# NUS-HPC-AI-Lab/VideoSys

Hardware: AMD Instinct MI355X
Metric: videos/min (Open-Sora 512x512x64f, 30 denoise steps, DiT denoising only) + sec/denoise-step (higher is better)
Workload: dtype bf16

## Files before the change

### videosys_amd/csrc/gemm2_bf16.hip

```cpp
#include "common.h"
#include "vsys_internal.h"

namespace vsys {
namespace {

constexpr int BM = 256, BK = 32;
constexpr int A_SLOT = BM * BK * 2;
constexpr int W_BASE = 3 * A_SLOT;
constexpr int OUT_ROW_BYTES = 96 * 2 + 16;
constexpr int OUT_WAVE_BYTES = 64 * OUT_ROW_BYTES;

template <int NWN>
struct G2 {
  static constexpr int NW = 2 * NWN;
  static constexpr int NT = 64 * NW;
  static constexpr int BN = 96 * NWN;
  static constexpr int NA = 16 / NW;
  static constexpr int W_SLOT = BN * BK * 2;
  static constexpr int WLEAD = NWN == 4 ? 2 : 1;
  static constexpr int NWSLOT = WLEAD + 1;
  static constexpr int STAGING = W_BASE + NWSLOT * W_SLOT;
  static constexpr int LDS_BYTES = STAGING > NW * OUT_WAVE_BYTES ? STAGING : NW * OUT_WAVE_BYTES;
  static constexpr int LN_BYTES = (BM + BN) * 8;
};

template <int EPI, int NWN, int STAMP = 0, int MF = 0>
__global__ __launch_bounds__(G2<NWN>::NT, 2) void gemm2_kernel(GemmParams p) {
  using G = G2<NWN>;
  constexpr int BN = G::BN, NA = G::NA, W_SLOT = G::W_SLOT, WLEAD = G::WLEAD;
#if __HIP_DEVICE_COMPILE__
  extern __shared__ __attribute__((aligned(16))) char smem[];
  const int tid = threadIdx.x, lane = tid & 63, wave = tid >> 6;
  const int wm = wave / NWN, wn = wave % NWN;
  const int l31 = lane & 31, hi = lane >> 5;
  const int l15 = lane & 15, lq = lane >> 4;
  static_assert(!MF || (EPI != EPI_F32_SLICES && !STAMP), "the 16x16x32 form covers the token-row epilogues only");
  const int wave_u = __builtin_amdgcn_readfirstlane(wave);
  const int nbn = p.N / BN;
  int tile = xcd_remap(blockIdx.x, gridDim.x);
  int kslice = 0;
  if constexpr (EPI == EPI_F32_SLICES) {
    const int ntile = ((p.M + BM - 1) / BM) * nbn;
    kslice = tile / ntile;
    tile -= kslice * ntile;
  }
  int bm, bn;
  gemm_raster(tile, (p.M + BM - 1) / BM, nbn, p.raster_gw, p.raster_ph, bm, bn);
  const int row0 = bm * BM, col0 = bn * BN;

  const int dchunk = ((lane & 3) ^ (MF ? ((0x78 >> (2 * ((lane >> 4) & 3))) & 3) : ((lane >> 4) & 3))) * 16;
  int a_off[NA], b_off[3];
#pragma unroll
  for (int i = 0; i < NA; ++i) {
    const int r = wave_u * (16 * NA) + i * 16 + (lane >> 2);
    const int rl = row0 + r < p.M ? r : p.M - 1 - row0;
    a_off[i] = rl * (int)p.lda * 2 + dchunk;
  }
#pragma unroll
  for (int i = 0; i < 3; ++i) b_off[i] = (wave_u * 48 + i * 16 + (lane >> 2)) * (int)p.ldw * 2 + dchunk;
  const int64_t a_bytes = ((int64_t)(p.M - 1 - row0) * p.lda + p.K) * 2, b_bytes = ((int64_t)(p.N - 1 - col0) * p.ldw + p.K) * 2;
  const auto rsrc_a = __builtin_amdgcn_make_buffer_rsrc((void*)(p.A + (int64_t)row0 * p.lda), 0,
                                                        (int)(a_bytes < 0x7fffffff ? a_bytes : 0x7fffffff), 0x00020000);
  const auto rsrc_b = __builtin_amdgcn_make_buffer_rsrc((void*)(p.W + (int64_t)col0 * p.ldw), 0,
                                                        (int)(b_bytes < 0x7fffffff ? b_bytes : 0x7fffffff), 0x00020000);
  typedef __attribute__((address_space(3))) void* lds_ptr_t;
  const int kbase2 = EPI == EPI_F32_SLICES ? kslice * p.ks * 2 : 0;
  auto dma_a = [&](int i, int t, int slot) {
    __builtin_amdgcn_raw_ptr_buffer_load_lds(rsrc_a, (lds_ptr_t)(smem + slot * A_SLOT + (wave_u * (16 * NA) + i * 16) * 64), 16, a_off[i],
                                             kbase2 + t * (BK * 2), 0, 0);
  };
  auto dma_w = [&](int i, int t, int slot) {
    __builtin_amdgcn_raw_ptr_buffer_load_lds(rsrc_b, (lds_ptr_t)(smem + W_BASE + slot * W_SLOT + (wave_u * 48 + i * 16) * 64), 16,
                                             b_off[i], kbase2 + t * (BK * 2), 0, 0);
  };

  const int fsw = MF ? ((lq ^ ((0x78 >> (2 * ((l15 >> 2) & 3))) & 3)) << 4) : ((hi ^ ((l31 >> 2) & 3)) << 4);
  const int frow = MF ? l15 : l31;
  const int xo = (wm * 128 + frow) * 64 + fsw;
  const int wo = W_BASE + (wn * 96 + frow) * 64 + fsw;

  f32x16 acc[MF ? 1 : 4][MF ? 1 : 3];
  f32x4 acc16[MF ? 8 : 1][MF ? 6 : 1];
#pragma unroll
  for (int i = 0; i < (MF ? 1 : 4); ++i)
#pragma unroll
    for (int j = 0; j < (MF ? 1 : 3); ++j)
#pragma unroll
      for (int r = 0; r < 16; ++r) acc[i][j][r] = 0.f;
#pragma unroll
  for (int i = 0; i < (MF ? 8 : 1); ++i)
#pragma unroll
    for (int j = 0; j < (MF ? 6 : 1); ++j)
#pragma unroll
      for (int r = 0; r < 4; ++r) acc16[i][j][r] = 0.f;

  constexpr bool LN = EPI == EPI_LN_BIAS || EPI == EPI_LN_GELU;
  float2* ln_lds = reinterpret_cast<float2*>(smem + G::LDS_BYTES);
  const int nt = (EPI == EPI_F32_SLICES ? (p.ks < p.K - kslice * p.ks ? p.ks : p.K - kslice * p.ks) : p.K) / BK;
#pragma unroll
  for (int i = 0; i < NA; ++i) dma_a(i, 0, 0);
#pragma unroll
  for (int i = 0; i < 3; ++i) dma_w(i, 0, 0);
  if (nt > 1) {
#pragma unroll
    for (int i = 0; i < NA; ++i) dma_a(i, 1, 1);
    if constexpr (WLEAD == 2) {
#pragma unroll
      for (int i = 0; i < 3; ++i) dma_w(i, 1, 1);
    }
  }
  if constexpr (LN) {
    __builtin_amdgcn_sched_barrier(0);
    ln_stage_tile(ln_lds, p.ln_stats, p.ln_ld, p.ln_nb, p.ln_eps, p.M, row0, BM, p.cs, p.cv, col0, BN, tid, G::NT);
    __builtin_amdgcn_sched_barrier(0);
  }
  if (nt > 1) {
    if constexpr (WLEAD == 2) {
      asm volatile("s_waitcnt vmcnt(5)" ::: "memory");
    } else if constexpr (NA == 4) {
      asm volatile("s_waitcnt vmcnt(4)" ::: "memory");
    } else {
      asm volatile("s_waitcnt vmcnt(2)" ::: "memory");
    }
  } else {
    asm volatile("s_waitcnt vmcnt(0)" ::: "memory");
  }
  if constexpr (LN) asm volatile("s_waitcnt lgkmcnt(0)" ::: "memory");
  __builtin_amdgcn_sched_barrier(0);
  __builtin_amdgcn_s_barrier();
  __builtin_amdgcn_sched_barrier(0);

  int sa = 0, sw = 0;
  uint64_t st_read = 0, st_mfma = 0, st_wait = 0, st_bar = 0, st_t0 = 0, st_begin = 0;
  if constexpr (STAMP) { st_begin = __builtin_amdgcn_s_memtime(); st_t0 = st_begin; }
  for (int t = 0; t < nt; ++t) {
    const int sa1 = sa == 2 ? 0 : sa + 1, sa2 = sa1 == 2 ? 0 : sa1 + 1;
    const int sw1 = WLEAD == 2 ? sa1 : (sw ^ 1);
    const int swn = WLEAD == 2 ? sa2 : sw1;
    const int tw = t + WLEAD;
    const bool n2 = t + 2 < nt;
    const bool n1 = WLEAD == 2 ? n2 : (t + 1 < nt);
    const char* ab = smem + sa * A_SLOT;
    const char* wb = smem + sw * W_SLOT;
    bf16x8 x0, x1, x2, x3, w0, w1, w2, v0, v1, v2;
    if constexpr (MF) {
      x0 = *reinterpret_cast<const bf16x8*>(ab + xo);
      w0 = *reinterpret_cast<const bf16x8*>(wb + wo);
      w1 = *reinterpret_cast<const bf16x8*>(wb + wo + 1024);
      w2 = *reinterpret_cast<const bf16x8*>(wb + wo + 2048);
      v0 = *reinterpret_cast<const bf16x8*>(wb + wo + 3072);
      v1 = *reinterpret_cast<const bf16x8*>(wb + wo + 4096);
      v2 = *reinterpret_cast<const bf16x8*>(wb + wo + 5120);
      x1 = *reinterpret_cast<const bf16x8*>(ab + xo + 1024);
      x2 = *reinterpret_cast<const bf16x8*>(ab + xo + 2048);
      x3 = *reinterpret_cast<const bf16x8*>(ab + xo + 3072);
      __builtin_amdgcn_sched_barrier(0);
#define G16_ROW(i_, X_)                                                                                \
  acc16[i_][0] = __builtin_amdgcn_mfma_f32_16x16x32_bf16(w0, X_, acc16[i_][0], 0, 0, 0);               \
  acc16[i_][1] = __builtin_amdgcn_mfma_f32_16x16x32_bf16(w1, X_, acc16[i_][1], 0, 0, 0);               \
  acc16[i_][2] = __builtin_amdgcn_mfma_f32_16x16x32_bf16(w2, X_, acc16[i_][2], 0, 0, 0);               \
  acc16[i_][3] = __builtin_amdgcn_mfma_f32_16x16x32_bf16(v0, X_, acc16[i_][3], 0, 0, 0);               \
  acc16[i_][4] = __builtin_amdgcn_mfma_f32_16x16x32_bf16(v1, X_, acc16[i_][4], 0, 0, 0);               \
  acc16[i_][5] = __builtin_amdgcn_mfma_f32_16x16x32_bf16(v2, X_, acc16[i_][5], 0, 0, 0)
      G16_ROW(0, x0);
      __builtin_amdgcn_sched_barrier(0);
      x0 = *reinterpret_cast<const bf16x8*>(ab + xo + 4096);
      if (n1) { dma_w(0, tw, swn); dma_w(1, tw, swn); }
      __builtin_amdgcn_sched_barrier(0);
      G16_ROW(1, x1);
      __builtin_amdgcn_sched_barrier(0);
      x1 = *reinterpret_cast<const bf16x8*>(ab + xo + 5120);
      if (n1) dma_w(2, tw, swn);
      if (n2) dma_a(0, t + 2, sa2);
      __builtin_amdgcn_sched_barrier(0);
      G16_ROW(2, x2);
      __builtin_amdgcn_sched_barrier(0);
      x2 = *reinterpret_cast<const bf16x8*>(ab + xo + 6144);
      if (n2) {
        dma_a(1, t + 2, sa2);
        if constexpr (NA > 2) dma_a(2 < NA ? 2 : 0, t + 2, sa2);
      }
      __builtin_amdgcn_sched_barrier(0);
      G16_ROW(3, x3);
      __builtin_amdgcn_sched_barrier(0);
      x3 = *reinterpret_cast<const bf16x8*>(ab + xo + 7168);
      if constexpr (NA > 3) {
        if (n2) dma_a(3 < NA ? 3 : 0, t + 2, sa2);
      }
      __builtin_amdgcn_sched_barrier(0);
      G16_ROW(4, x0);
      G16_ROW(5, x1);
      G16_ROW(6, x2);
      G16_ROW(7, x3);
#undef G16_ROW
    } else {
    x0 = *reinterpret_cast<const bf16x8*>(ab + xo);
    w0 = *reinterpret_cast<const bf16x8*>(wb + wo);
    w1 = *reinterpret_cast<const bf16x8*>(wb + wo + 2048);
    w2 = *reinterpret_cast<const bf16x8*>(wb + wo + 4096);
    x1 = *reinterpret_cast<const bf16x8*>(ab + xo + 2048);
    x2 = *reinterpret_cast<const bf16x8*>(ab + xo + 4096);
    x3 = *reinterpret_cast<const bf16x8*>(ab + xo + 6144);
    v0 = *reinterpret_cast<const bf16x8*>(wb + (wo ^ 32));
    v1 = *reinterpret_cast<const bf16x8*>(wb + (wo ^ 32) + 2048);
    v2 = *reinterpret_cast<const bf16x8*>(wb + (wo ^ 32) + 4096);
    __builtin_amdgcn_sched_barrier(0);
    if constexpr (STAMP) {
      asm volatile("s_waitcnt lgkmcnt(0)" ::: "memory");
      const uint64_t now = __builtin_amdgcn_s_memtime();
      st_read += now - st_t0; st_t0 = now;
      __builtin_amdgcn_sched_barrier(0);
    }
#define G2_ROW(i_, X_, W0_, W1_, W2_)                                                                  \
  acc[i_][0] = __builtin_amdgcn_mfma_f32_32x32x16_bf16(W0_, X_, acc[i_][0], 0, 0, 0);                  \
  acc[i_][1] = __builtin_amdgcn_mfma_f32_32x32x16_bf16(W1_, X_, acc[i_][1], 0, 0, 0);                  \
  acc[i_][2] = __builtin_amdgcn_mfma_f32_32x32x16_bf16(W2_, X_, acc[i_][2], 0, 0, 0)
    G2_ROW(0, x0, w0, w1, w2);
    __builtin_amdgcn_sched_barrier(0);
    x0 = *reinterpret_cast<const bf16x8*>(ab + (xo ^ 32));
    if (n1) { dma_w(0, tw, swn); dma_w(1, tw, swn); }
    __builtin_amdgcn_sched_barrier(0);
    G2_ROW(1, x1, w0, w1, w2);
    __builtin_amdgcn_sched_barrier(0);
    x1 = *reinterpret_cast<const bf16x8*>(ab + (xo ^ 32) + 2048);
    if (n1) dma_w(2, tw, swn);
    if (n2) dma_a(0, t + 2, sa2);
    __builtin_amdgcn_sched_barrier(0);
    G2_ROW(2, x2, w0, w1, w2);
    __builtin_amdgcn_sched_barrier(0);
    x2 = *reinterpret_cast<const bf16x8*>(ab + (xo ^ 32) + 4096);
    if (n2) {
      dma_a(1, t + 2, sa2);
      if constexpr (NA > 2) dma_a(2 < NA ? 2 : 0, t + 2, sa2);
    }
    __builtin_amdgcn_sched_barrier(0);
    G2_ROW(3, x3, w0, w1, w2);
    __builtin_amdgcn_sched_barrier(0);
    x3 = *reinterpret_cast<const bf16x8*>(ab + (xo ^ 32) + 6144);
    if constexpr (NA > 3) {
      if (n2) dma_a(3 < NA ? 3 : 0, t + 2, sa2);
    }
    __builtin_amdgcn_sched_barrier(0);
    G2_ROW(0, x0, v0, v1, v2);
    G2_ROW(1, x1, v0, v1, v2);
    G2_ROW(2, x2, v0, v1, v2);
    G2_ROW(3, x3, v0, v1, v2);
#undef G2_ROW
    }
    __builtin_amdgcn_sched_barrier(0);
    if constexpr (STAMP) {
      const uint64_t now = __builtin_amdgcn_s_memtime();
      st_mfma += now - st_t0; st_t0 = now;
      __builtin_amdgcn_sched_barrier(0);
    }
    if (n2) {
      if constexpr (WLEAD == 2) asm volatile("s_waitcnt vmcnt(5) lgkmcnt(0)" ::: "memory");
      else if constexpr (NA == 4) asm volatile("s_waitcnt vmcnt(4) lgkmcnt(0)" ::: "memory");
      else asm volatile("s_waitcnt vmcnt(2) lgkmcnt(0)" ::: "memory");
    } else {
      asm volatile("s_waitcnt vmcnt(0) lgkmcnt(0)" ::: "memory");
    }
    __builtin_amdgcn_sched_barrier(0);
    if constexpr (STAMP) {
      const uint64_t now = __builtin_amdgcn_s_memtime();
      st_wait += now - st_t0; st_t0 = now;
      __builtin_amdgcn_sched_barrier(0);
    }
    __builtin_amdgcn_s_barrier();
    __builtin_amdgcn_sched_barrier(0);
    if constexpr (STAMP) {
      const uint64_t now = __builtin_amdgcn_s_memtime();
      st_bar += now - st_t0; st_t0 = now;
      __builtin_amdgcn_sched_barrier(0);
    }
    sa = sa1;
    sw = sw1;
  }

  if constexpr (EPI == EPI_F32_SLICES) {
    float* o32 = p.out32 + (int64_t)kslice * p.slab;
    const int ncol0 = col0 + wn * 96;
#pragma unroll
    for (int i = 0; i < 4; ++i) {
      const int n = row0 + wm * 128 + i * 32 + l31;
      if (n < p.M) {
#pragma unroll
        for (int j = 0; j < 3; ++j)
#pragma unroll
          for (int g = 0; g < 4; ++g)
#pragma unroll
            for (int r = 0; r < 4; ++r) {
              const int m = ncol0 + j * 32 + 8 * g + 4 * hi + r;
              if (m < p.rows_per_sample) o32[(int64_t)m * p.ldo32 + n] = acc[i][j][4 * g + r];
            }
      }
    }
    return;
  }
  char* st = smem + wave * OUT_WAVE_BYTES;
  const int ncol0 = col0 + wn * 96;
  uint2 bb[3][4];
#pragma unroll
  for (int j = 0; j < 3; ++j)
#pragma unroll
    for (int g = 0; g < 4; ++g) bb[j][g] = make_uint2(0, 0);
  if (p.bias != nullptr && EPI != EPI_LN_BIAS && EPI != EPI_LN_GELU && !MF) {
#pragma unroll
    for (int j = 0; j < 3; ++j)
#pragma unroll
      for (int g = 0; g < 4; ++g) bb[j][g] = *reinterpret_cast<const uint2*>(p.bias + ncol0 + j * 32 + 8 * g + 4 * hi);
  }
  uint2 bb16[6];
#pragma unroll
  for (int j = 0; j < 6; ++j) bb16[j] = make_uint2(0, 0);
  if (MF && p.bias != nullptr && EPI != EPI_LN_BIAS && EPI != EPI_LN_GELU) {
#pragma unroll
    for (int j = 0; j < 6; ++j) bb16[j] = *reinterpret_cast<const uint2*>(p.bias + ncol0 + j * 16 + 4 * lq);
  }
  const bool full = row0 + BM <= p.M;
#pragma unroll
  for (int ih = 0; ih < 2; ++ih) {
    const int wrow0 = row0 + wm * 128 + ih * 64;
    if constexpr (MF) {
      if constexpr (LN) {
        float mu[4], rs[4];
#pragma unroll
        for (int i2 = 0; i2 < 4; ++i2) {
          const float2 ms = ln_lds[wm * 128 + ih * 64 + i2 * 16 + l15];
          mu[i2] = ms.x;
          rs[i2] = ms.y;
        }
#pragma unroll
        for (int j = 0; j < 6; ++j) {
          const float4* cp = reinterpret_cast<const float4*>(ln_lds + BM + wn * 96 + j * 16 + 4 * lq);
          const float4 a = cp[0], b = cp[1];
          const float c_s[4] = {a.x, a.z, b.x, b.z}, c_v[4] = {a.y, a.w, b.y, b.w};
#pragma unroll
          for (int i2 = 0; i2 < 4; ++i2) {
            const int i = ih * 4 + i2;
            const float nmu = -mu[i2], r_ = rs[i2];
            float v[4];
#pragma unroll
            for (int r = 0; r < 4; ++r) v[r] = fmaf(r_, fmaf(nmu, c_s[r], acc16[i][j][r]), c_v[r]);
            if (EPI == EPI_LN_GELU) {
#pragma unroll
              for (int r = 0; r < 4; ++r) v[r] = gelu_tanh(v[r]);
            }
            uint2 o;
            o.x = pack2bf(v[0], v[1]);
            o.y = pack2bf(v[2], v[3]);
            *reinterpret_cast<uint2*>(st + (i2 * 16 + l15) * OUT_ROW_BYTES + (j * 16 + 4 * lq) * 2) = o;
          }
        }
      } else {
        constexpr bool GATED16 = EPI == EPI_GATE_RES || EPI == EPI_GATE_RES_STATS;
        if (GATED16 && p.res != nullptr) {
#pragma unroll
          for (int half = 0; half < 2; ++half) {
            uint4 r6[6];
#pragma unroll
            for (int k = 0; k < 6; ++k) {
              const int q = lane + 64 * (6 * half + k);
              const int m_local = q / 12, c = q - m_local * 12;
              int grow = wrow0 + m_local;
              grow = grow < p.M ? grow : p.M - 1;
              r6[k] = *reinterpret_cast<const uint4*>(p.res + (int64_t)grow * p.ldr + ncol0 + c * 8);
            }
#pragma unroll
            for (int k = 0; k < 6; ++k) {
              const int q = lane + 64 * (6 * half + k);
              const int m_local = q / 12, c = q - m_local * 12;
              *reinterpret_cast<uint4*>(st + m_local * OUT_ROW_BYTES + c * 16) = r6[k];
            }
          }
          asm volatile("s_waitcnt lgkmcnt(0)" ::: "memory");
          __builtin_amdgcn_wave_barrier();
        }
#pragma unroll
        for (int i2 = 0; i2 < 4; ++i2) {
          const int i = ih * 4 + i2;
          const int m_local = i2 * 16 + l15;
          const bf16_t* gate_row = nullptr;
          if (GATED16 && p.gate != nullptr) {
            int grow = wrow0 + m_local;
            grow = grow < p.M ? grow : p.M - 1;
            const int sample = grow / p.rows_per_sample;
            gate_row = p.gate + (int64_t)sample * p.gate_stride + ncol0 + 4 * lq;
            if (p.seg_split > 0 && grow - sample * p.rows_per_sample < p.seg_split) gate_row += p.gate_alt;
          }
#pragma unroll
          for (int j = 0; j < 6; ++j) {
            uint2 gg = make_uint2(0x3f803f80u, 0x3f803f80u);
            if (GATED16 && gate_row != nullptr) gg = *reinterpret_cast<const uint2*>(gate_row + j * 16);
            float v[4];
#pragma unroll
            for (int r = 0; r < 4; ++r) v[r] = acc16[i][j][r];
            v[0] += bflo(bb16[j].x); v[1] += bfhi(bb16[j].x); v[2] += bflo(bb16[j].y); v[3] += bfhi(bb16[j].y);
            if (EPI == EPI_BIAS_GELU) {
#pragma unroll
              for (int r = 0; r < 4; ++r) v[r] = gelu_tanh(v[r]);
            }
            if (GATED16) {
              v[0] *= bflo(gg.x); v[1] *= bfhi(gg.x); v[2] *= bflo(gg.y); v[3] *= bfhi(gg.y);
            }
            uint2 o;
            o.x = pack2bf(v[0], v[1]);
            o.y = pack2bf(v[2], v[3]);
            if (GATED16 && p.res != nullptr) {
              const uint2 rr = *reinterpret_cast<const uint2*>(st + m_local * OUT_ROW_BYTES + (j * 16 + 4 * lq) * 2);
              o.x = pack2bf(bflo(o.x) + bflo(rr.x), bfhi(o.x) + bfhi(rr.x));
              o.y = pack2bf(bflo(o.y) + bflo(rr.y), bfhi(o.y) + bfhi(rr.y));
            }
            *reinterpret_cast<uint2*>(st + m_local * OUT_ROW_BYTES + (j * 16 + 4 * lq) * 2) = o;
          }
        }
        if constexpr (EPI == EPI_GATE_RES_STATS) {
          asm volatile("s_waitcnt lgkmcnt(0)" ::: "memory");
          __builtin_amdgcn_wave_barrier();
#pragma unroll
          for (int i2 = 0; i2 < 2; ++i2) {
            const int m_local = i2 * 32 + l31;
            LnAcc lacc;
#pragma unroll
            for (int j = 0; j < 3; ++j)
#pragma unroll
              for (int g = 0; g < 4; ++g) {
                const uint2 o = *reinterpret_cast<const uint2*>(st + m_local * OUT_ROW_BYTES + (j * 32 + 8 * g + 4 * hi) * 2);
                if (j == 0 && g == 0) lacc.init(bflo(o.x));
                lacc.add(bflo(o.x)); lacc.add(bfhi(o.x)); lacc.add(bflo(o.y)); lacc.add(bfhi(o.y));
              }
            const float2 mine = lacc.finish(48.f);
            const float2 other = make_float2(__shfl_xor(mine.x, 32, 64), __shfl_xor(mine.y, 32, 64));
            const float2 blk = ln_merge_equal(mine, other, 48.f);
            const int grow = wrow0 + m_local;
            if (hi == 0 && grow < p.M) p.stats_out[(int64_t)(ncol0 / LN_BLOCK) * p.stats_ld + grow] = blk;
          }
        }
      }
    } else {
    if constexpr (LN) {
      float mu[2], rs[2];
#pragma unroll
      for (int i2 = 0; i2 < 2; ++i2) {
        const float2 ms = ln_lds[wm * 128 + ih * 64 + i2 * 32 + l31];
        mu[i2] = ms.x;
        rs[i2] = ms.y;
      }
#pragma unroll
      for (int j = 0; j < 3; ++j) {
        float4 c_s[4], c_v[4];
#pragma unroll
        for (int g = 0; g < 4; ++g) {
          const float4* cp = reinterpret_cast<const float4*>(ln_lds + BM + wn * 96 + j * 32 + 8 * g + 4 * hi);
          const float4 a = cp[0], b = cp[1];
          c_s[g] = make_float4(a.x, a.z, b.x, b.z);
          c_v[g] = make_float4(a.y, a.w, b.y, b.w);
        }
#pragma unroll
        for (int i2 = 0; i2 < 2; ++i2) {
          const int i = ih * 2 + i2;
          const int m_local = i2 * 32 + l31;
          const float nmu = -mu[i2], r_ = rs[i2];
#pragma unroll
          for (int g = 0; g < 4; ++g) {
            const int n_local = j * 32 + 8 * g + 4 * hi;
            float v[4];
            v[0] = fmaf(r_, fmaf(nmu, c_s[g].x, acc[i][j][4 * g + 0]), c_v[g].x);
            v[1] = fmaf(r_, fmaf(nmu, c_s[g].y, acc[i][j][4 * g + 1]), c_v[g].y);
            v[2] = fmaf(r_, fmaf(nmu, c_s[g].z, acc[i][j][4 * g + 2]), c_v[g].z);
            v[3] = fmaf(r_, fmaf(nmu, c_s[g].w, acc[i][j][4 * g + 3]), c_v[g].w);
            if (EPI == EPI_LN_GELU) {
#pragma unroll
              for (int r = 0; r < 4; ++r) v[r] = gelu_tanh(v[r]);
            }
            uint2 o;
            o.x = pack2bf(v[0], v[1]);
            o.y = pack2bf(v[2], v[3]);
            *reinterpret_cast<uint2*>(st + m_local * OUT_ROW_BYTES + n_local * 2) = o;
          }
        }
      }
    }
#pragma unroll
    for (int i2 = 0; i2 < (LN ? 0 : 2); ++i2) {
      const int i = ih * 2 + i2;
      const int m_local = i2 * 32 + l31;
      const bf16_t* gate_row = nullptr;
      if (EPI == EPI_GATE_RES && p.gate != nullptr) {
        int grow = wrow0 + m_local;
        grow = grow < p.M ? grow : p.M - 1;
        const int sample = grow / p.rows_per_sample;
        gate_row = p.gate + (int64_t)sample * p.gate_stride + ncol0 + 4 * hi;
        if (p.seg_split > 0 && grow - sample * p.rows_per_sample < p.seg_split) gate_row += p.gate_alt;
      }
#pragma unroll
      for (int j = 0; j < 3; ++j) {
        uint2 gg[4];
        if (EPI == EPI_GATE_RES) {
#pragma unroll
          for (int g = 0; g < 4; ++g) gg[g] = make_uint2(0x3f803f80u, 0x3f803f80u);
          if (gate_row != nullptr) {
#pragma unroll
            for (int g = 0; g < 4; ++g) gg[g] = *reinterpret_cast<const uint2*>(gate_row + j * 32 + 8 * g);
          }
        }
#pragma unroll
        for (int g = 0; g < 4; ++g) {
          const int n_local = j * 32 + 8 * g + 4 * hi;
          float v[4];
#pragma unroll
          for (int r = 0; r < 4; ++r) v[r] = acc[i][j][4 * g + r];
          v[0] += bflo(bb[j][g].x); v[1] += bfhi(bb[j][g].x); v[2] += bflo(bb[j][g].y); v[3] += bfhi(bb[j][g].y);
          if (EPI == EPI_BIAS_GELU) {
#pragma unroll
            for (int r = 0; r < 4; ++r) v[r] = gelu_tanh(v[r]);
          }
          if (EPI == EPI_GATE_RES) {
            v[0] *= bflo(gg[g].x); v[1] *= bfhi(gg[g].x); v[2] *= bflo(gg[g].y); v[3] *= bfhi(gg[g].y);
          }
          uint2 o;
          o.x = pack2bf(v[0], v[1]);
          o.y = pack2bf(v[2], v[3]);
          *reinterpret_cast<uint2*>(st + m_local * OUT_ROW_BYTES + n_local * 2) = o;
        }
      }
    }
    }
    uint4 rres[12];
    if (EPI == EPI_GATE_RES && !MF) {
#pragma unroll
      for (int it = 0; it < 12; ++it) rres[it] = make_uint4(0, 0, 0, 0);
      if (p.res != nullptr) {
#pragma unroll
        for (int it = 0; it < 12; ++it) {
          const int q = lane + 64 * it;
          const int m_local = q / 12, c = q - m_local * 12;
          int grow = wrow0 + m_local;
          grow = grow < p.M ? grow : p.M - 1;
          rres[it] = *reinterpret_cast<const uint4*>(p.res + (int64_t)grow * p.ldr + ncol0 + c * 8);
        }
      }
    }
    asm volatile("s_waitcnt lgkmcnt(0)" ::: "memory");
    __builtin_amdgcn_wave_barrier();
    uint4 val[12];
#pragma unroll
    for (int it = 0; it < 12; ++it) {
      const int q = lane + 64 * it;
      const int m_local = q / 12, c = q - m_local * 12;
      val[it] = *reinterpret_cast<const uint4*>(st + m_local * OUT_ROW_BYTES + c * 16);
    }
#pragma unroll
    for (int it = 0; it < 12; ++it) {
      const int q = lane + 64 * it;
      const int m_local = q / 12, c = q - m_local * 12;
      const int64_t grow = wrow0 + m_local;
      const int gcol = ncol0 + c * 8;
      const bool ok = full || grow < p.M;
      uint4 v = val[it];
      if (EPI == EPI_GATE_RES && !MF) {
        if (p.aux != nullptr && ok) *reinterpret_cast<uint4*>(p.aux + grow * p.ldaux + gcol) = v;
        if (p.res != nullptr) {
          float a[8], b[8];
          unpack8(v, a);
          unpack8(rres[it], b);
#pragma unroll
          for (int e = 0; e < 8; ++e) a[e] += b[e];
          v = pack8(a);
        }
      }
      if (ok) *reinterpret_cast<uint4*>(p.out + grow * p.ldo + gcol) = v;
    }
    asm volatile("s_waitcnt lgkmcnt(0)" ::: "memory");
    __builtin_amdgcn_wave_barrier();
  }
  if constexpr (STAMP) {
    if (lane == 0 && p.aux != nullptr) {
      int64_t* d = reinterpret_cast<int64_t*>(p.aux) + ((int64_t)blockIdx.x * G::NW + wave) * 8;
      const uint64_t end = __builtin_amdgcn_s_memtime();
      d[0] = (int64_t)st_read; d[1] = (int64_t)st_mfma; d[2] = (int64_t)st_wait; d[3] = (int64_t)st_bar;
      d[4] = (int64_t)(st_t0 - st_begin); d[5] = (int64_t)(end - st_t0); d[6] = (int64_t)st_begin; d[7] = nt;
    }
  }
#endif
}

}

template <int NWN, int MF = 0>
static int launch_gemm2_t(const GemmParams& p, int epi, hipStream_t stream) {
  using G = G2<NWN>;
  if (p.N % G::BN != 0) return VSYS_ERR_SHAPE;
  const int nbm = (p.M + BM - 1) / BM, nbn = p.N / G::BN;
  const int grid = nbm * nbn;
  static std::atomic<unsigned long long> attr_seen{0};
  for (DeviceOnce once(attr_seen); once.todo(); once.done()) {
    (void)hipFuncSetAttribute((const void*)gemm2_kernel<EPI_BIAS, NWN, 0, MF>, hipFuncAttributeMaxDynamicSharedMemorySize, G::LDS_BYTES);
    (void)hipFuncSetAttribute((const void*)gemm2_kernel<EPI_BIAS_GELU, NWN, 0, MF>, hipFuncAttributeMaxDynamicSharedMemorySize, G::LDS_BYTES);
    (void)hipFuncSetAttribute((const void*)gemm2_kernel<EPI_GATE_RES, NWN, 0, MF>, hipFuncAttributeMaxDynamicSharedMemorySize, G::LDS_BYTES);
    (void)hipFuncSetAttribute((const void*)gemm2_kernel<EPI_LN_BIAS, NWN, 0, MF>, hipFuncAttributeMaxDynamicSharedMemorySize, G::LDS_BYTES + G::LN_BYTES);
    (void)hipFuncSetAttribute((const void*)gemm2_kernel<EPI_LN_GELU, NWN, 0, MF>, hipFuncAttributeMaxDynamicSharedMemorySize, G::LDS_BYTES + G::LN_BYTES);
    if constexpr (MF)
      (void)hipFuncSetAttribute((const void*)gemm2_kernel<EPI_GATE_RES_STATS, NWN, 0, MF>, hipFuncAttributeMaxDynamicSharedMemorySize, G::LDS_BYTES);
  }
  switch (epi) {
    case EPI_LN_BIAS: hipLaunchKernelGGL((gemm2_kernel<EPI_LN_BIAS, NWN, 0, MF>), dim3(grid), dim3(G::NT), G::LDS_BYTES + G::LN_BYTES, stream, p); break;
    case EPI_LN_GELU: hipLaunchKernelGGL((gemm2_kernel<EPI_LN_GELU, NWN, 0, MF>), dim3(grid), dim3(G::NT), G::LDS_BYTES + G::LN_BYTES, stream, p); break;
    case EPI_BIAS: hipLaunchKernelGGL((gemm2_kernel<EPI_BIAS, NWN, 0, MF>), dim3(grid), dim3(G::NT), G::LDS_BYTES, stream, p); break;
    case EPI_BIAS_GELU: hipLaunchKernelGGL((gemm2_kernel<EPI_BIAS_GELU, NWN, 0, MF>), dim3(grid), dim3(G::NT), G::LDS_BYTES, stream, p); break;
    case EPI_GATE_RES:
      if (MF && (p.aux || p.add1 || p.add2 || p.stats_out)) return VSYS_ERR_ARG;
      hipLaunchKernelGGL((gemm2_kernel<EPI_GATE_RES, NWN, 0, MF>), dim3(grid), dim3(G::NT), G::LDS_BYTES, stream, p); break;
    case EPI_GATE_RES_STATS:
      if constexpr (MF) {
        hipLaunchKernelGGL((gemm2_kernel<EPI_GATE_RES_STATS, NWN, 0, MF>), dim3(grid), dim3(G::NT), G::LDS_BYTES, stream, p);
        break;
      }
      return VSYS_ERR_ARG;
    default: return VSYS_ERR_ARG;
  }
  return hipGetLastError() == hipSuccess ? 0 : VSYS_ERR_LAUNCH;
}

#ifdef VSYS_LAB
int launch_gemm2_stamp(const GemmParams& p_, hipStream_t stream) {
  using G = G2<4>;
  GemmParams p = p_;
  p.aux = reinterpret_cast<bf16_t*>(get_lab_debug_buffer());
  if (p.N % G::BN != 0 || p.aux == nullptr) return VSYS_ERR_SHAPE;
  const int grid = ((p.M + BM - 1) / BM) * (p.N / G::BN);
  (void)hipFuncSetAttribute((const void*)gemm2_kernel<EPI_BIAS, 4, 1>, hipFuncAttributeMaxDynamicSharedMemorySize, G::LDS_BYTES);
  hipLaunchKernelGGL((gemm2_kernel<EPI_BIAS, 4, 1>), dim3(grid), dim3(G::NT), G::LDS_BYTES, stream, p);
  return hipGetLastError() == hipSuccess ? 0 : VSYS_ERR_LAUNCH;
}

#endif

int launch_gemm2_slices(const GemmParams& p, int slices, hipStream_t stream) {
  using G = G2<4>;
  if (p.M <= 0) return 0;
  if (p.N % G::BN != 0 || slices < 1 || slices > 65535 || p.ks <= 0 || p.ks % BK != 0 || p.K % BK != 0 || (int64_t)p.ks * slices < p.K ||
      (int64_t)p.ks * (slices - 1) >= p.K || p.out32 == nullptr || (p.lda % 8) || (p.ldw % 8) || p.rows_per_sample <= 0)
    return VSYS_ERR_SHAPE;
  if (p.lda * 512 + (int64_t)p.K * 2 >= 0x7fffffff || p.ldw * 768 + (int64_t)p.K * 2 >= 0x7fffffff) return VSYS_ERR_SHAPE;
  const int nbm = (p.M + BM - 1) / BM, nbn = p.N / G::BN;
  static std::atomic<unsigned long long> attr_seen{0};
  for (DeviceOnce once(attr_seen); once.todo(); once.done())
    (void)hipFuncSetAttribute((const void*)gemm2_kernel<EPI_F32_SLICES, 4>, hipFuncAttributeMaxDynamicSharedMemorySize, G::LDS_BYTES);
  hipLaunchKernelGGL((gemm2_kernel<EPI_F32_SLICES, 4>), dim3(nbm * nbn * slices), dim3(G::NT), G::LDS_BYTES, stream, p);
  return hipGetLastError() == hipSuccess ? 0 : VSYS_ERR_LAUNCH;
}

int launch_gemm2(const GemmParams& p, int epi, int wide, hipStream_t stream) {
  if (wide == 2) return launch_gemm2_t<2, 1>(p, epi, stream);
  if (wide == 3) return launch_gemm2_t<4, 1>(p, epi, stream);
  return wide ? launch_gemm2_t<4>(p, epi, stream) : launch_gemm2_t<2>(p, epi, stream);
}

}
```

### videosys_amd/csrc/gemm_bf16.hip

```cpp
#include <map>
#include <mutex>

#include "common.h"
#include "vsys_internal.h"

namespace vsys {

namespace {

constexpr int BN = 192, BK = 64;
constexpr int B_BYTES = BN * BK * 2;
constexpr int OUT_ROW_BYTES = 96 * 2 + 16;
constexpr int OUT_WAVE_BYTES = 64 * OUT_ROW_BYTES;

template <int BM_>
struct Geo {
  static constexpr int NW = BM_ / 32;
  static constexpr int NT = NW * 64;
  static constexpr int A_BYTES = BM_ * BK * 2;
  static constexpr int STAGE = A_BYTES + B_BYTES;
  static constexpr int NA = 4;
  static constexpr int NB = BN / NW / 8;
  static_assert(NW * OUT_WAVE_BYTES <= 2 * STAGE, "epilogue image must fit in the staging buffers");
};
// ... 922 lines not shown
    const bool ok = grow < p.M;
    if (EPI == EPI_GATE_RES) {
      if (p.aux != nullptr && ok) *reinterpret_cast<uint4*>(p.aux + (int64_t)grow * p.ldaux + gcol) = val;
      if (p.res != nullptr) {
        float a[8], b[8];
        unpack8(val, a);
        unpack8(rres[it], b);
#pragma unroll
        for (int e = 0; e < 8; ++e) a[e] += b[e];
        val = pack8(a);
      }
    }
    if (ok) *reinterpret_cast<uint4*>(p.out + (int64_t)grow * p.ldo + gcol) = val;
  }
#endif
}

__global__ __launch_bounds__(256) void linear_small_kernel(const bf16_t* __restrict__ x, int64_t ldx,
                                                           const bf16_t* __restrict__ w, int64_t ldw,
                                                           const bf16_t* __restrict__ bias, bf16_t* __restrict__ out,
                                                           int64_t ldo, int M, int N, int K, int act_in, int act_out) {
  const int wave = threadIdx.x >> 6, lane = threadIdx.x & 63;
  const int64_t idx = (int64_t)blockIdx.x * 4 + wave;
  if (idx >= (int64_t)M * N) return;
  const int m = (int)(idx / N), n = (int)(idx - (int64_t)m * N);
  const bf16_t* xr = x + (int64_t)m * ldx;
  const bf16_t* wr = w + (int64_t)n * ldw;
  float s = 0.f;
  for (int k = lane * 8; k < K; k += 64 * 8) {
    uint4 xv = *reinterpret_cast<const uint4*>(xr + k);
    uint4 wv = *reinterpret_cast<const uint4*>(wr + k);
    float a[8], b[8];
    unpack8(xv, a);
    unpack8(wv, b);
#pragma unroll
    for (int e = 0; e < 8; ++e) {
      float xe = a[e];
      if (act_in == ACT_SILU) xe = bf2f(f2bf(silu(xe)));
      s += xe * b[e];
    }
  }
  s = wave_sum(s);
  if (lane == 0) {
    if (bias != nullptr) s += bf2f(bias[n]);
    if (act_out == ACT_SILU) s = silu(s);
    else if (act_out == ACT_GELU_TANH) s = gelu_tanh(s);
    out[(int64_t)m * ldo + n] = f2bf(s);
  }
}

}

static std::atomic<int> g_gemm_variant_a{0};
static std::atomic<int> g_gemm_raster_a{600};
int set_gemm_variant(int v) {
  if (v >= 20000 && v < 30000) {
    g_gemm_raster_a.store(v - 20000, std::memory_order_relaxed);
    return 0;
  }
  switch (v) {
    case 0: case 3: case 6: case 8: case 9: case 16: case 20: case 24: case 34: case 28: case 30: case 50: case 103: case 106: case 113: case 118: case 119: case 123: break;
#ifdef VSYS_LAB
    case 60: case 70: case 80:
    case 18: case 38: case 48: case 31: case 40: case 61: case 62: case 63: case 64: case 71: case 72: case 73: case 74: case 78: case 81: case 82: case 83: case 84: break;
#endif
    default: return VSYS_ERR_ARG;
  }
  g_gemm_variant_a.store(v, std::memory_order_relaxed);
  return 0;
}

template <int PIPE, int BM_, int RASTER = 1, int PROD = 0, int MF = 0, int KS = 0>
static int launch_gemm_t(const GemmParams& p, int epi, hipStream_t stream) {
  using G = Geo<BM_>;
  if (PROD && epi != EPI_BIAS && epi != EPI_BIAS_GELU) return launch_gemm_t<PIPE, BM_, RASTER, 0, MF, KS>(p, epi, stream);
  const int nbm = (p.M + BM_ - 1) / BM_, nbn = p.N / BN;
  const int grid = KS ? ((nbm * nbn + 7) / 8) * 16 : nbm * nbn;
  const bool lnl = epi == EPI_LN_BIAS || epi == EPI_LN_GELU;
  const size_t lds = ((PIPE % 10 == 8) ? 3 * G::A_BYTES + 2 * B_BYTES : (PIPE % 10 == 9 ? 3 : 2) * G::STAGE) + (lnl && BM_ == 256 ? (BM_ + BN) * 8 : 0);
  static std::atomic<unsigned long long> attr_seen{0};
  for (DeviceOnce once(attr_seen); once.todo(); once.done()) {
    const int lds = (int)(((PIPE % 10 == 8) ? 3 * G::A_BYTES + 2 * B_BYTES : (PIPE % 10 == 9 ? 3 : 2) * G::STAGE) + (BM_ == 256 ? (BM_ + BN) * 8 : 0));
    (void)hipFuncSetAttribute((const void*)gemm_kernel<EPI_BIAS, PIPE, BM_, RASTER, PROD, MF, KS>, hipFuncAttributeMaxDynamicSharedMemorySize, (int)lds);
    (void)hipFuncSetAttribute((const void*)gemm_kernel<EPI_BIAS_GELU, PIPE, BM_, RASTER, PROD, MF, KS>, hipFuncAttributeMaxDynamicSharedMemorySize, (int)lds);
    (void)hipFuncSetAttribute((const void*)gemm_kernel<EPI_GATE_RES, PIPE, BM_, RASTER, 0, MF, KS>, hipFuncAttributeMaxDynamicSharedMemorySize, (int)lds);
    if constexpr (!PROD) {
      (void)hipFuncSetAttribute((const void*)gemm_kernel<EPI_GATE_RES_STATS, PIPE, BM_, RASTER, 0, MF, KS>, hipFuncAttributeMaxDynamicSharedMemorySize, (int)lds);
      (void)hipFuncSetAttribute((const void*)gemm_kernel<EPI_LN_BIAS, PIPE, BM_, RASTER, 0, MF, KS>, hipFuncAttributeMaxDynamicSharedMemorySize, (int)lds);
      (void)hipFuncSetAttribute((const void*)gemm_kernel<EPI_LN_GELU, PIPE, BM_, RASTER, 0, MF, KS>, hipFuncAttributeMaxDynamicSharedMemorySize, (int)lds);
    }
  }
  constexpr int NTH = G::NT + PROD * 256;
  switch (epi) {
    case EPI_BIAS: hipLaunchKernelGGL((gemm_kernel<EPI_BIAS, PIPE, BM_, RASTER, PROD, MF, KS>), dim3(grid), dim3(NTH), lds, stream, p); break;
    case EPI_BIAS_GELU: hipLaunchKernelGGL((gemm_kernel<EPI_BIAS_GELU, PIPE, BM_, RASTER, PROD, MF, KS>), dim3(grid), dim3(NTH), lds, stream, p); break;
    case EPI_GATE_RES: hipLaunchKernelGGL((gemm_kernel<EPI_GATE_RES, PIPE, BM_, RASTER, 0, MF, KS>), dim3(grid), dim3(G::NT), lds, stream, p); break;
    case EPI_GATE_RES_STATS: hipLaunchKernelGGL((gemm_kernel<EPI_GATE_RES_STATS, PIPE, BM_, RASTER, 0, MF, KS>), dim3(grid), dim3(G::NT), lds, stream, p); break;
    case EPI_LN_BIAS: hipLaunchKernelGGL((gemm_kernel<EPI_LN_BIAS, PIPE, BM_, RASTER, 0, MF, KS>), dim3(grid), dim3(G::NT), lds, stream, p); break;
    case EPI_LN_GELU: hipLaunchKernelGGL((gemm_kernel<EPI_LN_GELU, PIPE, BM_, RASTER, 0, MF, KS>), dim3(grid), dim3(G::NT), lds, stream, p); break;
    default: return VSYS_ERR_ARG;
  }
  return hipGetLastError() == hipSuccess ? 0 : VSYS_ERR_LAUNCH;
}

static bool mf16_default() {
  static const bool on = [] { const char* e = getenv("VSYS_GEMM_MF16"); return !(e && e[0] == '0'); }();
  return on;
}

namespace {
struct SplitKWs { float* ws = nullptr; int* flags = nullptr; int tiles = 0; };
std::mutex g_splitk_mutex;
std::map<hipStream_t, SplitKWs> g_splitk_ws;
}
static bool splitk_workspace(hipStream_t stream, int tiles, GemmParams& p) {
  std::lock_guard<std::mutex> lock(g_splitk_mutex);
  SplitKWs& w = g_splitk_ws[stream];
  if (w.ws == nullptr) {
    const int cap = cu_count_this_device();
    hipStreamCaptureStatus cs = hipStreamCaptureStatusNone;
    if (hipStreamIsCapturing(stream, &cs) == hipSuccess && cs != hipStreamCaptureStatusNone) return false;
    if (hipMalloc(&w.ws, (size_t)cap * 4 * 24 * 64 * sizeof(float4)) != hipSuccess) { w.ws = nullptr; return false; }
    if (hipMalloc(&w.flags, (size_t)cap * 4 * sizeof(int)) != hipSuccess || hipMemset(w.flags, 0, (size_t)cap * 4 * sizeof(int)) != hipSuccess) {
      (void)hipFree(w.ws);
      w.ws = nullptr;
      return false;
    }
    (void)hipDeviceSynchronize();
    w.tiles = cap;
  }
  if (tiles > w.tiles) return false;
  p.sk_ws = w.ws;
  p.sk_flags = w.flags;
  return true;
}
static int launch_rows128(const GemmParams& p_, int epi, hipStream_t stream, bool force_split = false) {
  if (!mf16_default() && !force_split) return launch_gemm_t<3, 128>(p_, epi, stream);
  static const bool splitk_on = [] { const char* e = getenv("VSYS_GEMM_SPLITK"); return e && e[0] == '1'; }();
  const int tiles = ((p_.M + 127) / 128) * (p_.N / BN);
  if ((splitk_on || force_split) && tiles >= 64 && tiles <= cu_count_this_device() && p_.K / BK >= 8) {
    GemmParams p = p_;
    if (splitk_workspace(stream, tiles, p)) return launch_gemm_t<3, 128, 1, 0, 1, 1>(p, epi, stream);
  }
  static const bool s8_on = [] { const char* e = getenv("VSYS_GEMM_ROWS128_S8"); return e && e[0] == '1'; }();
  if (s8_on && tiles <= cu_count_this_device() && p_.K / BK >= 3) return launch_gemm_t<8, 128, 1, 0, 1>(p_, epi, stream);
  static const bool ring_off = [] { const char* e = getenv("VSYS_GEMM_ROWS128_RING"); return e && e[0] == '0'; }();
  if (!ring_off && tiles <= cu_count_this_device() && p_.K / BK >= 3) return launch_gemm_t<9, 128, 1, 0, 1>(p_, epi, stream);
  return launch_gemm_t<3, 128, 1, 0, 1>(p_, epi, stream);
}
static int launch_sched8(const GemmParams& p, int epi, hipStream_t stream) {
  return mf16_default() ? launch_gemm_t<8, 256, 1, 0, 1>(p, epi, stream) : launch_gemm_t<8, 256>(p, epi, stream);
}

int launch_gemm(const GemmParams& p_, int epi, hipStream_t stream) {
  if (p_.M <= 0) return 0;
  GemmParams p = p_;
  {
    const int ras = g_gemm_raster_a.load(std::memory_order_relaxed);
    p.raster_gw = ras / 100;
    p.raster_ph = ras % 100;
  }
  if (p.N % BN != 0 || p.K % BK != 0 || p.N <= 0 || p.K <= 0) return VSYS_ERR_SHAPE;
  if ((p.lda % 8) || (p.ldw % 8) || (p.ldo % 8) || (p.res && (p.ldr % 8)) || (p.aux && (p.ldaux % 8))) return VSYS_ERR_ALIGN;
  if (p.lda * 512 + (int64_t)p.K * 2 >= 0x7fffffff || p.ldw * 384 + (int64_t)p.K * 2 >= 0x7fffffff) return VSYS_ERR_SHAPE;
  if ((epi == EPI_GATE_RES || epi == EPI_GATE_RES_STATS) && p.gate && p.rows_per_sample <= 0) return VSYS_ERR_SHAPE;
  const bool ln = epi == EPI_LN_BIAS || epi == EPI_LN_GELU;
  if (ln && (!p.cs || !p.cv || !p.ln_stats || p.ln_nb < 1 || p.ln_nb > 12 || p.ln_nb * LN_BLOCK != p.K || p.ln_ld < p.M)) return VSYS_ERR_SHAPE;
  if (epi == EPI_GATE_RES_STATS && (!p.stats_out || p.stats_ld < p.M || p.aux)) return VSYS_ERR_ARG;
  if (epi != EPI_GATE_RES && (p.add1 || p.add2)) return VSYS_ERR_ARG;
  if (epi == EPI_GATE_RES && (p.add1 || p.add2 || p.stats_out)) {
    if ((p.add2 && !p.add1) || ((p.add1 || p.add2) && (!p.res || (p.ldr % 8))) || (p.stats_out && p.stats_ld < p.M)) return VSYS_ERR_ARG;
    if ((int64_t)((p.M + 255) / 256) * (p.N / BN) < 400) return launch_rows128(p, epi, stream, g_gemm_variant_a.load(std::memory_order_relaxed) == 123);
    return g_gemm_variant_a.load(std::memory_order_relaxed) == 8 ? launch_gemm_t<8, 256>(p, epi, stream) : launch_sched8(p, epi, stream);
  }
  if (epi == EPI_GATE_RES_STATS) {
    if ((int64_t)((p.M + 255) / 256) * (p.N / BN) < 400) return launch_rows128(p, epi, stream, g_gemm_variant_a.load(std::memory_order_relaxed) == 123);
    if (g_gemm_variant_a.load(std::memory_order_relaxed) == 24) return launch_gemm2(p, epi, 2, stream);
    return g_gemm_variant_a.load(std::memory_order_relaxed) == 8 ? launch_gemm_t<8, 256>(p, epi, stream) : launch_sched8(p, epi, stream);
  }
  if (ln) {
    if ((int64_t)((p.M + 255) / 256) * (p.N / BN) < 400) return launch_rows128(p, epi, stream, g_gemm_variant_a.load(std::memory_order_relaxed) == 123);
    if (p.K <= 1536 && p.N >= 2304 && g_gemm_variant_a.load(std::memory_order_relaxed) != 8) return launch_gemm2(p, epi, mf16_default() ? 2 : 0, stream);
    return g_gemm_variant_a.load(std::memory_order_relaxed) == 8 ? launch_gemm_t<8, 256>(p, epi, stream) : launch_sched8(p, epi, stream);
  }
  const int g_gemm_variant = g_gemm_variant_a.load(std::memory_order_relaxed);
  switch (g_gemm_variant == 50 ? 0 : g_gemm_variant) {
    case 6: return launch_gemm_t<6, 256>(p, epi, stream);
#ifdef VSYS_LAB
    case 18: return launch_gemm_t<18, 256>(p, epi, stream);
    case 48: return launch_gemm_t<48, 256>(p, epi, stream);
    case 38: return launch_gemm_t<38, 256>(p, epi, stream);
    case 40: return launch_gemm3(p, epi, stream);
    case 31: return (epi == EPI_BIAS && p.N % 384 == 0) ? launch_gemm2_stamp(p, stream) : VSYS_ERR_ARG;
    case 61: case 62: case 63: case 64: return epi == EPI_BIAS ? launch_gemm4_lab(p, g_gemm_variant - 60, 0, stream) : VSYS_ERR_ARG;
    case 71: case 72: case 73: case 74: case 78: return epi == EPI_BIAS ? launch_gemm4_lab(p, g_gemm_variant - 70, 1, stream) : VSYS_ERR_ARG;
    case 60: case 70: case 80:
      if (!gemm4_supports(p, epi)) return launch_gemm_t<8, 256>(p, epi, stream);
      return launch_gemm4(p, epi, (g_gemm_variant - 60) / 10, stream);
    case 81: case 82: case 83: case 84:
      return gemm4_supports(p, epi) ? launch_gemm4(p, epi, 2 + g_gemm_variant - 80, stream) : VSYS_ERR_ARG;
#endif
    case 103: return launch_gemm_t<3, 128>(p, epi, stream);
    case 113: return launch_gemm_t<3, 128, 1, 0, 1>(p, epi, stream);
    case 118: return launch_gemm_t<8, 128, 1, 0, 1>(p, epi, stream);
    case 119: return launch_gemm_t<9, 128, 1, 0, 1>(p, epi, stream);
    case 123: return launch_rows128(p, epi, stream, true);
    case 106: return launch_gemm_t<6, 128>(p, epi, stream);
    case 20: return launch_gemm2(p, epi, 0, stream);
    case 24:
      if (epi == EPI_GATE_RES && p.aux) return launch_sched8(p, epi, stream);
      return launch_gemm2(p, epi, 2, stream);
    case 30: return p.N % 384 == 0 ? launch_gemm2(p, epi, 1, stream) : launch_gemm_t<8, 256>(p, epi, stream);
    case 34: return (p.N % 384 == 0 && !(epi == EPI_GATE_RES && p.aux)) ? launch_gemm2(p, epi, 3, stream) : launch_sched8(p, epi, stream);
    case 8: return launch_gemm_t<8, 256>(p, epi, stream);
    case 16: return launch_gemm_t<8, 256, 1, 0, 1>(p, epi, stream);
    case 28: return launch_gemm_t<8, 256, 1, 1>(p, epi, stream);
    case 3: return launch_gemm_t<3, 256>(p, epi, stream);
    case 9: return launch_gemm_t<8, 256, 0>(p, epi, stream);
    default:
      if ((int64_t)((p.M + 255) / 256) * (p.N / BN) < 400) return launch_rows128(p, epi, stream, g_gemm_variant_a.load(std::memory_order_relaxed) == 123);
      if (epi != EPI_GATE_RES && p.K <= 1536 && mf16_default()) return launch_gemm2(p, epi, 2, stream);
      if (epi != EPI_GATE_RES && p.K <= 1536 && p.N >= 2304) return launch_gemm2(p, epi, 0, stream);
      if (g_gemm_variant == 50 && p.K >= 2304 && p.N % 384 == 0) return launch_gemm2(p, epi, 1, stream);
      return launch_sched8(p, epi, stream);
  }
}

int launch_linear_small(const bf16_t* x, int64_t ldx, const bf16_t* w, int64_t ldw, const bf16_t* bias, bf16_t* out,
                        int64_t ldo, int M, int N, int K, int act_in, int act_out, hipStream_t stream) {
  if (M <= 0 || N <= 0) return 0;
  if (K % 8 != 0 || (ldx % 8) || (ldw % 8)) return VSYS_ERR_ALIGN;
  const int64_t total = (int64_t)M * N;
  const int64_t grid = (total + 3) / 4;
  if (grid > 0x7fffffff) return VSYS_ERR_SHAPE;
  hipLaunchKernelGGL(linear_small_kernel, dim3((unsigned)grid), dim3(256), 0, stream, x, ldx, w, ldw, bias, out, ldo, M, N,
                     K, act_in, act_out);
  return hipGetLastError() == hipSuccess ? 0 : VSYS_ERR_LAUNCH;
}

}
```

Baseline: 20.72.

## Stream residual tile into LDS via buffer DMA and route gated GEMMs to gemm2

In the MFMA gemm2 epilogue for the gated-residual variants, the residual tile is now loaded with buffer_load-to-LDS DMA into a swizzled LDS image. The first half is issued before the epilogue and the second half overlaps with the first half's stores. The per-row gate loads are replaced by a single per-tile gate load when the tile lies within one sample. The dispatcher now sends gated-residual and gated-residual-stats GEMMs with K≤1536 to gemm2 by default instead of sched8. This adds shape guards against 32-bit buffer offset overflow and changes the LDS layout, which the stats and store paths have to match.

```diff
diff --git a/videosys_amd/csrc/gemm2_bf16.hip b/videosys_amd/csrc/gemm2_bf16.hip
--- a/videosys_amd/csrc/gemm2_bf16.hip
+++ b/videosys_amd/csrc/gemm2_bf16.hip
@@ -130,6 +130,16 @@
   __builtin_amdgcn_s_barrier();
   __builtin_amdgcn_sched_barrier(0);
 
+  constexpr bool GATED_MF = MF && (EPI == EPI_GATE_RES || EPI == EPI_GATE_RES_STATS);
+  const int64_t r_bytes = GATED_MF ? ((int64_t)(p.M - 1 - row0) * p.ldr + p.N - col0) * 2 : 0;
+  const auto rsrc_r = __builtin_amdgcn_make_buffer_rsrc((void*)(GATED_MF && p.res ? p.res + (int64_t)row0 * p.ldr + col0 : p.res), 0,
+                                                        (int)(r_bytes < 0x7fffffff ? r_bytes : 0x7fffffff), 0x00020000);
+  auto res_voff = [&](int kk) {
+    const int q = 64 * (kk & 63) + lane, m = q / 12, c = (q - 12 * m) ^ ((m >> 2) & 3);
+    int r = wm * 128 + (kk >> 6) * 64 + m;
+    r = row0 + r < p.M ? r : p.M - 1 - row0;
+    return r * (int)p.ldr * 2 + (wn * 96 + c * 8) * 2;
+  };
   int sa = 0, sw = 0;
   uint64_t st_read = 0, st_mfma = 0, st_wait = 0, st_bar = 0, st_t0 = 0, st_begin = 0;
   if constexpr (STAMP) { st_begin = __builtin_amdgcn_s_memtime(); st_t0 = st_begin; }
@@ -318,6 +328,33 @@
     for (int j = 0; j < 6; ++j) bb16[j] = *reinterpret_cast<const uint2*>(p.bias + ncol0 + j * 16 + 4 * lq);
   }
   const bool full = row0 + BM <= p.M;
+  constexpr int SROW = 192, SWAVE = 64 * SROW;
+  constexpr bool SPLIT = GATED_MF && G::NW * (SWAVE + 32 * SROW) <= G::LDS_BYTES;
+  char* const s_a = smem + wave_u * SWAVE;
+  char* const s_b = smem + G::NW * SWAVE + wave_u * (32 * SROW);
+  auto img = [&](int ih_, int m_lo) -> char* { return (SPLIT && ih_ == 1 && m_lo < 32) ? s_b : s_a; };
+  const bool resd = GATED_MF && p.res != nullptr;
+  auto dma_res = [&](int ih_, int k) {
+    __builtin_amdgcn_raw_ptr_buffer_load_lds(rsrc_r, (lds_ptr_t)(img(ih_, k < 6 ? 0 : 32) + k * 1024), 16, res_voff(64 * ih_ + k), 0, 0, 0);
+  };
+  uint2 gt[6];
+  bool gate_tile = false;
+  if constexpr (GATED_MF) {
+    if (resd) {
+#pragma unroll
+      for (int k = 0; k < 12; ++k) dma_res(0, k);
+      if constexpr (SPLIT) {
+#pragma unroll
+        for (int k = 0; k < 6; ++k) dma_res(1, k);
+      }
+    }
+    gate_tile = p.gate != nullptr && p.seg_split <= 0 && p.rows_per_sample % BM == 0;
+    if (gate_tile) {
+      const bf16_t* g0 = p.gate + (int64_t)(row0 / p.rows_per_sample) * p.gate_stride + ncol0 + 4 * lq;
+#pragma unroll
+      for (int j = 0; j < 6; ++j) gt[j] = *reinterpret_cast<const uint2*>(g0 + j * 16);
+    }
+  }
 #pragma unroll
   for (int ih = 0; ih < 2; ++ih) {
     const int wrow0 = row0 + wm * 128 + ih * 64;
@@ -353,35 +390,20 @@
           }
         }
       } else {
-        constexpr bool GATED16 = EPI == EPI_GATE_RES || EPI == EPI_GATE_RES_STATS;
-        if (GATED16 && p.res != nullptr) {
-#pragma unroll
-          for (int half = 0; half < 2; ++half) {
-            uint4 r6[6];
-#pragma unroll
-            for (int k = 0; k < 6; ++k) {
-              const int q = lane + 64 * (6 * half + k);
-              const int m_local = q / 12, c = q - m_local * 12;
-              int grow = wrow0 + m_local;
-              grow = grow < p.M ? grow : p.M - 1;
-              r6[k] = *reinterpret_cast<const uint4*>(p.res + (int64_t)grow * p.ldr + ncol0 + c * 8);
-            }
-#pragma unroll
-            for (int k = 0; k < 6; ++k) {
-              const int q = lane + 64 * (6 * half + k);
-              const int m_local = q / 12, c = q - m_local * 12;
-              *reinterpret_cast<uint4*>(st + m_local * OUT_ROW_BYTES + c * 16) = r6[k];
-            }
-          }
-          asm volatile("s_waitcnt lgkmcnt(0)" ::: "memory");
-          __builtin_amdgcn_wave_barrier();
-        }
+        constexpr bool GATED16 = GATED_MF;
+        const int sx = (l15 >> 2) & 3, cq = lq >> 1;
+        auto eptr = [&](int i2, int j) -> char* {
+          if constexpr (GATED16) return img(ih, i2 * 16) + (i2 * 16 + l15) * SROW + ((((2 * j) | cq) ^ sx) << 4) + 8 * (lq & 1);
+          else return st + (i2 * 16 + l15) * OUT_ROW_BYTES + (j * 16 + 4 * lq) * 2;
+        };
+        if (resd && ih == 0) asm volatile("s_waitcnt vmcnt(0)" ::: "memory");
 #pragma unroll
         for (int i2 = 0; i2 < 4; ++i2) {
           const int i = ih * 4 + i2;
           const int m_local = i2 * 16 + l15;
+          if (resd && ih == 1 && i2 == (SPLIT ? 2 : 0)) asm volatile("s_waitcnt vmcnt(0)" ::: "memory");
           const bf16_t* gate_row = nullptr;
-          if (GATED16 && p.gate != nullptr) {
+          if (GATED16 && p.gate != nullptr && !gate_tile) {
             int grow = wrow0 + m_local;
             grow = grow < p.M ? grow : p.M - 1;
             const int sample = grow / p.rows_per_sample;
@@ -391,7 +413,8 @@
 #pragma unroll
           for (int j = 0; j < 6; ++j) {
             uint2 gg = make_uint2(0x3f803f80u, 0x3f803f80u);
-            if (GATED16 && gate_row != nullptr) gg = *reinterpret_cast<const uint2*>(gate_row + j * 16);
+            if (GATED16 && gate_tile) gg = gt[j];
+            else if (GATED16 && gate_row != nullptr) gg = *reinterpret_cast<const uint2*>(gate_row + j * 16);
             float v[4];
 #pragma unroll
             for (int r = 0; r < 4; ++r) v[r] = acc16[i][j][r];
@@ -406,12 +429,12 @@
             uint2 o;
             o.x = pack2bf(v[0], v[1]);
             o.y = pack2bf(v[2], v[3]);
-            if (GATED16 && p.res != nullptr) {
-              const uint2 rr = *reinterpret_cast<const uint2*>(st + m_local * OUT_ROW_BYTES + (j * 16 + 4 * lq) * 2);
+            if (resd) {
+              const uint2 rr = *reinterpret_cast<const uint2*>(eptr(i2, j));
               o.x = pack2bf(bflo(o.x) + bflo(rr.x), bfhi(o.x) + bfhi(rr.x));
               o.y = pack2bf(bflo(o.y) + bflo(rr.y), bfhi(o.y) + bfhi(rr.y));
             }
-            *reinterpret_cast<uint2*>(st + m_local * OUT_ROW_BYTES + (j * 16 + 4 * lq) * 2) = o;
+            *reinterpret_cast<uint2*>(eptr(i2, j)) = o;
           }
         }
         if constexpr (EPI == EPI_GATE_RES_STATS) {
@@ -425,7 +448,7 @@
             for (int j = 0; j < 3; ++j)
 #pragma unroll
               for (int g = 0; g < 4; ++g) {
-                const uint2 o = *reinterpret_cast<const uint2*>(st + m_local * OUT_ROW_BYTES + (j * 32 + 8 * g + 4 * hi) * 2);
+                const uint2 o = *reinterpret_cast<const uint2*>(img(ih, i2 * 32) + m_local * SROW + (((4 * j + g) ^ ((m_local >> 2) & 3)) << 4) + 8 * hi);
                 if (j == 0 && g == 0) lacc.init(bflo(o.x));
                 lacc.add(bflo(o.x)); lacc.add(bfhi(o.x)); lacc.add(bflo(o.y)); lacc.add(bfhi(o.y));
               }
@@ -548,12 +571,19 @@
     for (int it = 0; it < 12; ++it) {
       const int q = lane + 64 * it;
       const int m_local = q / 12, c = q - m_local * 12;
-      val[it] = *reinterpret_cast<const uint4*>(st + m_local * OUT_ROW_BYTES + c * 16);
+      if constexpr (GATED_MF) val[it] = *reinterpret_cast<const uint4*>(img(ih, it < 6 ? 0 : 32) + q * 16);
+      else val[it] = *reinterpret_cast<const uint4*>(st + m_local * OUT_ROW_BYTES + c * 16);
+    }
+    if (resd && ih == 0) {
+      asm volatile("s_waitcnt lgkmcnt(0)" ::: "memory");
+#pragma unroll
+      for (int k = SPLIT ? 6 : 0; k < 12; ++k) dma_res(1, k);
     }
 #pragma unroll
     for (int it = 0; it < 12; ++it) {
       const int q = lane + 64 * it;
-      const int m_local = q / 12, c = q - m_local * 12;
+      const int m_local = q / 12;
+      const int c = GATED_MF ? (q - m_local * 12) ^ ((m_local >> 2) & 3) : q - m_local * 12;
       const int64_t grow = wrow0 + m_local;
       const int gcol = ncol0 + c * 8;
       const bool ok = full || grow < p.M;
@@ -610,9 +640,11 @@
     case EPI_BIAS_GELU: hipLaunchKernelGGL((gemm2_kernel<EPI_BIAS_GELU, NWN, 0, MF>), dim3(grid), dim3(G::NT), G::LDS_BYTES, stream, p); break;
     case EPI_GATE_RES:
       if (MF && (p.aux || p.add1 || p.add2 || p.stats_out)) return VSYS_ERR_ARG;
+      if (MF && p.res && (int64_t)p.ldr * 512 + (int64_t)p.N * 2 >= 0x7fffffff) return VSYS_ERR_SHAPE;
       hipLaunchKernelGGL((gemm2_kernel<EPI_GATE_RES, NWN, 0, MF>), dim3(grid), dim3(G::NT), G::LDS_BYTES, stream, p); break;
     case EPI_GATE_RES_STATS:
       if constexpr (MF) {
+        if (p.res && (int64_t)p.ldr * 512 + (int64_t)p.N * 2 >= 0x7fffffff) return VSYS_ERR_SHAPE;
         hipLaunchKernelGGL((gemm2_kernel<EPI_GATE_RES_STATS, NWN, 0, MF>), dim3(grid), dim3(G::NT), G::LDS_BYTES, stream, p);
         break;
       }
diff --git a/videosys_amd/csrc/gemm_bf16.hip b/videosys_amd/csrc/gemm_bf16.hip
--- a/videosys_amd/csrc/gemm_bf16.hip
+++ b/videosys_amd/csrc/gemm_bf16.hip
@@ -1098,6 +1098,10 @@
   return mf16_default() ? launch_gemm_t<8, 256, 1, 0, 1>(p, epi, stream) : launch_gemm_t<8, 256>(p, epi, stream);
 }
 
+static bool gated_on_gemm2(const GemmParams& p) {
+  return mf16_default() && p.K <= 1536 && (!p.res || (int64_t)p.ldr * 512 + (int64_t)p.N * 2 < 0x7fffffff);
+}
+
 int launch_gemm(const GemmParams& p_, int epi, hipStream_t stream) {
   if (p_.M <= 0) return 0;
   GemmParams p = p_;
@@ -1121,8 +1125,11 @@
   }
   if (epi == EPI_GATE_RES_STATS) {
     if ((int64_t)((p.M + 255) / 256) * (p.N / BN) < 400) return launch_rows128(p, epi, stream, g_gemm_variant_a.load(std::memory_order_relaxed) == 123);
-    if (g_gemm_variant_a.load(std::memory_order_relaxed) == 24) return launch_gemm2(p, epi, 2, stream);
-    return g_gemm_variant_a.load(std::memory_order_relaxed) == 8 ? launch_gemm_t<8, 256>(p, epi, stream) : launch_sched8(p, epi, stream);
+    const int v = g_gemm_variant_a.load(std::memory_order_relaxed);
+    if (v == 24) return launch_gemm2(p, epi, 2, stream);
+    if (v == 8) return launch_gemm_t<8, 256>(p, epi, stream);
+    if (v == 16) return launch_gemm_t<8, 256, 1, 0, 1>(p, epi, stream);
+    return gated_on_gemm2(p) ? launch_gemm2(p, epi, 2, stream) : launch_sched8(p, epi, stream);
   }
   if (ln) {
     if ((int64_t)((p.M + 255) / 256) * (p.N / BN) < 400) return launch_rows128(p, epi, stream, g_gemm_variant_a.load(std::memory_order_relaxed) == 123);
@@ -1168,6 +1175,7 @@
       if (epi != EPI_GATE_RES && p.K <= 1536 && mf16_default()) return launch_gemm2(p, epi, 2, stream);
       if (epi != EPI_GATE_RES && p.K <= 1536 && p.N >= 2304) return launch_gemm2(p, epi, 0, stream);
       if (g_gemm_variant == 50 && p.K >= 2304 && p.N % 384 == 0) return launch_gemm2(p, epi, 1, stream);
+      if (epi == EPI_GATE_RES && !p.aux && gated_on_gemm2(p)) return launch_gemm2(p, epi, 2, stream);
       return launch_sched8(p, epi, stream);
   }
 }
```

Result: no change. 20.78 (median of 6 runs) (+0.3%).
